# prip-lab/MSU-LatentAFIS

Measured on AMD Instinct MI355X. Metric: latent queries/sec vs 100k rolled gallery, higher is better.
Workload: dtype f32

## Files before the change

### include/afis_matcher_taps.h

```cpp
#ifndef AFIS_MATCHER_TAPS_H
#define AFIS_MATCHER_TAPS_H

#include "afis_matcher.h"

#ifdef __cplusplus
extern "C" {
#endif

int afis_debug_lut(afis_ctx* ctx, const afis_template_view* query, float* out, int32_t* n_rows);
int afis_debug_texture_rowmax(afis_ctx* ctx, const afis_template_view* query, int64_t g,
                              float* val, int32_t* arg, int32_t* n_rows);

int afis_debug_stage_list(afis_ctx* ctx, const afis_template_view* query, int64_t g, int which, int stage,
                          float* sim, int32_t* li, int32_t* ri, int32_t* n);

int afis_debug_atan2_grid(afis_ctx* ctx, int R, float* out);

int afis_debug_graph_arith(afis_ctx* ctx, unsigned long long* out8);
int afis_debug_refine_stats(afis_ctx* ctx, unsigned long long* out8, int reset);

int afis_debug_compact_stats(afis_ctx* ctx, long long* out2);

int afis_debug_rank_subjects(afis_ctx* ctx, afis_subjects* subjects, const float* scores , int n_q, int k,
                             int64_t* subject_id, float* subject_score, int64_t* best_idx);

int afis_debug_rank_hits(afis_ctx* ctx, afis_subjects* subjects, const float* scores , int n_q, float min_score, int cap,
                         int64_t* n_hits , int64_t* out_a , float* out_score , int64_t* out_b );

int afis_debug_rank_latent_hits(afis_ctx* ctx, const float* scores , int n_q, float min_score, int cap, int64_t latent_base,
                                int64_t* n_hits , int64_t* latent_idx , float* score );
int afis_debug_rank_rows(afis_ctx* ctx, afis_subset* subset, const float* scores , int n_q, int k,
                         int64_t* topk_idx , float* topk_score );
int afis_debug_transpose_stats(afis_ctx* ctx, long long* out2);
int afis_debug_expand_rows(afis_ctx* ctx, const float* cls , int n_c, int64_t m, const int32_t* row_of , const int32_t* sel ,
                           int n_q, int64_t G, float* out );

int afis_debug_phase_cycles(afis_ctx* ctx, unsigned long long* out32, int reset);

#ifdef __cplusplus
}
#endif
#endif
```

### msu-latentafis_amd/csrc/afis_device.h

```cpp
#pragma once
#include <hip/hip_runtime.h>
#include <stdint.h>

#include "score_order.h"

namespace afis {

typedef unsigned long long u64;
constexpr int kM = 16;
constexpr int kK = 256;
constexpr int kDsub = 6;
constexpr int kDes = 96;
constexpr int kTexMax = 1000;
constexpr int kTopTex = 200;
constexpr int kTopMinu = 120;
constexpr int kDistN = 50;
constexpr int kTileRows = 8;
constexpr int kTileFloats = kTileRows * kM * kK;

struct GalleryDev {
    int32_t G = 0;
    const int32_t* minu_off = nullptr;
    const short2*  minu_xy = nullptr;
    const float*   minu_ori = nullptr;
// ... 86 lines not shown
AFIS_HOST_DEVICE constexpr int rt_class_keys_per_thread(int S) { return S == 4 ? 64 : 32; }
AFIS_HOST_DEVICE inline int rt_row_stride(int S, int nR) { return S == 1 ? (((nR & 1) || nR == 128) ? nR : nR + 1) : (nR | 1); }
AFIS_HOST_DEVICE inline int rt_max_rows(int S, int nR)
{
    if (nR <= 0 || nR > rt_class_max_rolled(S)) return 0;
    int m = rt_class_keys_per_thread(S) * ((256 * S) / nR);
    const int cap = rt_class_simi_floats(S) / rt_row_stride(S, nR);
    m = m < cap ? m : cap;
    return m < rt_class_max_latent(S) ? m : rt_class_max_latent(S);
}
inline long long launch_group_latents(long long G) { if (G < 1) G = 1; const long long w = (5000000 + G / 2) / G; return w < 10 ? 10 : w > 128 ? 128 : w; }
inline void launch_group_cuts(const long long* rows_prefix, int n, int per, bool by_row_groups, int* cuts , int* n_cuts)
{
    *n_cuts = 0;
    if (n <= 0) return;
    if (per < 1) per = 1;
    if (!by_row_groups || n == 1) { for (int i = per; i < n; i += per) cuts[(*n_cuts)++] = i; cuts[(*n_cuts)++] = n; return; }
    const long long kInf = 1ll << 60, rg_rows = 768;
    long long* best = new long long[(size_t)n + 1]; int* from = new int[(size_t)n + 1]; int* cnt = new int[(size_t)n + 1];
    best[0] = 0; from[0] = 0; cnt[0] = 0;
    for (int i = 1; i <= n; ++i) {
        best[i] = kInf; from[i] = 0; cnt[i] = 0;
        for (int j = (i - per > 0 ? i - per : 0); j < i; ++j) {
            const long long c = best[j] + (rows_prefix[i] - rows_prefix[j] + rg_rows - 1) / rg_rows;
            if (c < best[i] || (c == best[i] && cnt[j] + 1 < cnt[i])) { best[i] = c; from[i] = j; cnt[i] = cnt[j] + 1; }
        }
    }
    int m = 0;
    for (int i = n; i > 0; i = from[i]) cuts[m++] = i;
    for (int a = 0, b = m - 1; a < b; ++a, --b) { const int t = cuts[a]; cuts[a] = cuts[b]; cuts[b] = t; }
    *n_cuts = m;
    delete[] best; delete[] from; delete[] cnt;
}
inline size_t minu_fb_ints(size_t n_tasks, size_t G) { return 1 + n_tasks + 8 + 3 * G; }
inline size_t minu_scratch_floats(int max_nL, int max_nR, int s3_tie_order)
{
    const size_t n = ((size_t)(max_nL > 1 ? max_nL : 1) * (size_t)(max_nR > 1 ? max_nR : 1) + 63) / 64 * 64;
    return (s3_tie_order ? 5 : 2) * n + 4096;
}
enum { kDiagFallback = 0,
       kDiagSmall = 1,
       kDiagCandsClk = 4, kDiagCandsWall = 5,
       kDiagBoundClk = 6, kDiagBoundWall = 7,
       kDiagWords = 16 };
constexpr int kTexSlabSteps = 48, kMinuSlabSteps = 32;
constexpr size_t kTexSlabWgBytes = (size_t)((kTopTex + 63) / 64) * kTexSlabSteps * 64 * 5;
constexpr size_t kMinuSlabWgBytes = (size_t)((kTopMinu + 63) / 64) * kMinuSlabSteps * 64 * 5;
inline int graph_texture_grid(long long n_tasks) { return (int)(n_tasks < 16384 ? n_tasks : 16384); }
inline int graph_minutiae_grid(long long n_tasks) { return (int)(n_tasks < 32768 ? n_tasks : 32768); }
inline size_t graph_texture_slab_bytes(long long n_tasks) { return n_tasks > 0 ? (size_t)graph_texture_grid(n_tasks) * kTexSlabWgBytes : 0; }
inline size_t graph_minutiae_slab_bytes(long long n_tasks) { return n_tasks > 0 ? (size_t)graph_minutiae_grid(n_tasks) * kMinuSlabWgBytes : 0; }
hipError_t launch_graph_texture(const QueryDev& q, const GalleryDev& g, const float* table_dist,
                                const float* rm_val, const int32_t* rm_arg, const float* rm_cv, const int32_t* rm_n, float* parts, void* slab, size_t slab_bytes, MinuCand* tap_out, int32_t* tap_n, int tap_stage, hipStream_t stream);
hipError_t launch_minu_cands(const QueryDev& q, const GalleryDev& g, float* scratch, size_t scratch_floats_per_wg, int n_wg,
                             int force_generic, MinuCand* cands, int32_t* cand_n, int32_t* fallback , int max_nL, int max_nR,
                             unsigned long long* diag , hipStream_t stream);
hipError_t launch_graph_minutiae(const QueryDev& q, const GalleryDev& g, const MinuCand* cands, const int32_t* cand_n,
                                 float* parts, short4* corr_out, int32_t* corr_n, void* slab, size_t slab_bytes, MinuCand* tap_out, int32_t* tap_n, int tap_stage, hipStream_t stream, bool join = false);
hipError_t launch_fuse(const QueryDev& q, const GalleryDev& g, const float* parts, float* scores, hipStream_t stream);

hipError_t launch_topk(const float* scores, int n_q, int G, int k, long long index_base, long long* out_idx, float* out_score, hipStream_t stream);

hipError_t launch_pq_encode(const float* des, long long n, const float* codewords, uint8_t* codes, hipStream_t stream);
hipError_t launch_fragment_tiles(const float* des, const int32_t* off, const int32_t* tile_off, int n_templates, void* frag, hipStream_t stream);
hipError_t launch_compact_ranges(const void* src, void* dst, int elem_bytes, const int32_t* old_off, const int32_t* new_off, int G, long long n_new, hipStream_t stream);
hipError_t launch_gather_ranges(const void* src, void* dst, int elem_bytes, const int32_t* src_off, const int32_t* sel, const int32_t* dst_off, int n, long long n_out, hipStream_t stream);
hipError_t launch_subset_topk_map(long long* idx, long long n_idx, const long long* map, int n_map, hipStream_t stream);
// ... 40 lines not shown
```

### msu-latentafis_amd/csrc/afis_taps.cpp

```cpp
#include "afis_ctx.h"
#include "../../include/afis_matcher_taps.h"

using namespace afis;

static int ensure_codes_cf(afis_ctx* ctx, Shard& sh, int variant)
{
    if ((variant != 6 && variant != 7) || sh.codes_cf_built) return AFIS_OK;
    const int64_t G = sh.gal.G;
    std::vector<int32_t> to((size_t)G + 1), cfb((size_t)G + 1);
    HIPCHK(ctx, hipMemcpyAsync(to.data(), sh.gal.tex_off, to.size() * 4, hipMemcpyDeviceToHost, ctx->stream));
    HIPCHK(ctx, hipStreamSynchronize(ctx->stream));
    int64_t nblk = 0;
    for (int64_t t = 0; t < G; ++t) { cfb[(size_t)t] = (int32_t)nblk; const int64_t n = to[(size_t)t + 1] - to[(size_t)t]; nblk += n > 0 ? (n + 63) / 64 + 1 : 0; }
    cfb[(size_t)G] = (int32_t)nblk;
    if (nblk > 0x7fffffff / 64) return fail(ctx, AFIS_EINVAL, "adc_variant 6 / 7: shard too large for the direct kernel's code stream; split the gallery into more shards");
    HIPCHK(ctx, upload(sh.g_tex_cf_blk, cfb, ctx->stream));
    HIPCHK(ctx, sh.g_tex_codes_cf.ensure(std::max<size_t>((size_t)nblk * 64 * 16, 16)));
    sh.gal.tex_cf_blk = sh.g_tex_cf_blk.as<int32_t>();
    sh.gal.tex_codes_cf = sh.g_tex_codes_cf.as<uint4>();
    HIPCHK(ctx, launch_codes_cf(sh.gal, sh.g_tex_codes_cf.p, ctx->stream));
    HIPCHK(ctx, hipStreamSynchronize(ctx->stream));
    sh.codes_cf_built = true;
    return AFIS_OK;
}
// ... 279 lines not shown
            HIPCHK(ctx, ctx->rm_val.ensure((size_t)d.lt_pad * 4)); HIPCHK(ctx, ctx->rm_arg.ensure((size_t)d.lt_pad * 4));
            const int av = ctx->adc_variant >= 8 ? 0 : ctx->adc_variant;
            { int rcf = ensure_codes_cf(ctx, *ctx, av); if (rcf != AFIS_OK) return rcf; }
            if (av == 6 || av == 7) { one.tex_codes_cf = ctx->gal.tex_codes_cf; one.tex_cf_blk = ctx->gal.tex_cf_blk + gidx; }
            { int rcd = direct_rowmax(ctx, d, one, av, 32, nullptr); if (rcd != AFIS_OK) return rcd; }
            HIPCHK(ctx, ctx->tex_slab.ensure(graph_texture_slab_bytes(d.nq)));
            HIPCHK(ctx, launch_graph_texture(d, one, ctx->table.as<float>(), ctx->rm_val.as<float>(), ctx->rm_arg.as<int32_t>(), nullptr, nullptr, ctx->parts.as<float>(), ctx->tex_slab.p, ctx->tex_slab.bytes,
                                             d_out.as<MinuCand>(), d_n.as<int32_t>(), stage | (ctx->s89_tie_order << 8), s));
        } else {
            slot = which - 1; cap = kTopMinu;
            const size_t per_wg = minu_scratch_floats(grp.max_nL, ctx->max_nR, ctx->s3_tie_order);
            HIPCHK(ctx, ctx->scratch.ensure(per_wg * 4 * 64));
            HIPCHK(ctx, ctx->cands.ensure(3 * (size_t)kTopMinu * sizeof(MinuCand))); HIPCHK(ctx, ctx->cand_n.ensure(12)); HIPCHK(ctx, ctx->minu_fb.ensure(minu_fb_ints(3, 1) * 4));
            HIPCHK(ctx, launch_minu_cands(d, one, ctx->scratch.as<float>(), per_wg, 64, ctx->minu_generic | (ctx->s3_tie_order << 1), ctx->cands.as<MinuCand>(), ctx->cand_n.as<int32_t>(), ctx->minu_fb.as<int32_t>(), grp.max_nL, ctx->max_nR, nullptr, s));
            HIPCHK(ctx, ctx->minu_slab.ensure(graph_minutiae_slab_bytes(3ll * d.nq)));
            HIPCHK(ctx, launch_graph_minutiae(d, one, ctx->cands.as<MinuCand>(), ctx->cand_n.as<int32_t>(), ctx->parts.as<float>(), nullptr, nullptr, ctx->minu_slab.p, ctx->minu_slab.bytes,
                                              d_out.as<MinuCand>(), d_n.as<int32_t>(), stage | (ctx->s89_tie_order << 8), s));
        }
        std::vector<MinuCand> h((size_t)3 * kTopTex); int32_t hn[3] = {-1, -1, -1};
        HIPCHK(ctx, hipMemcpyAsync(h.data(), d_out.p, h.size() * sizeof(MinuCand), hipMemcpyDeviceToHost, s));
        HIPCHK(ctx, hipMemcpyAsync(hn, d_n.p, 12, hipMemcpyDeviceToHost, s));
        HIPCHK(ctx, hipStreamSynchronize(s));
        if (ctx->res_empty[(size_t)gidx]) return AFIS_OK;
        *n = hn[slot];
        for (int t = 0; t < hn[slot]; ++t) { const MinuCand& c = h[(size_t)slot * cap + t]; sim[t] = c.sim; li[t] = c.li; ri[t] = c.ri; }
        return AFIS_OK;
    };
    rc = body();
    d_out.release(); d_n.release(); grp.release();
    return rc;
}


}
```

### msu-latentafis_amd/csrc/minu.hip

```cpp
#include "afis_device.h"
#include "stdsort_order.h"
#include <cstdlib>

namespace afis {

constexpr int kThreads = 256;
constexpr int kWaves = kThreads / 64;

#ifdef AFIS_PHASE_TIMING
__device__ u64 g_phase_cycles[32];
#define PHASE_DECL() __shared__ u64 ph_acc[32]; if (threadIdx.x < 32) ph_acc[threadIdx.x] = 0; __syncthreads()
#define PHASE_FLUSH() do { __syncthreads(); if (threadIdx.x < 32 && ph_acc[threadIdx.x]) atomicAdd(&g_phase_cycles[threadIdx.x], ph_acc[threadIdx.x]); } while (0)
#define PHASE_INIT() u64 ph_t0 = __builtin_readcyclecounter()
#define PHASE(i) do { if (threadIdx.x == 0) { const u64 ph_t1 = __builtin_readcyclecounter(); ph_acc[i] += ph_t1 - ph_t0; ph_t0 = ph_t1; } } while (0)
#else
#define PHASE_DECL() do {} while (0)
#define PHASE_FLUSH() do {} while (0)
#define PHASE_INIT() do {} while (0)
#define PHASE(i) do {} while (0)
#endif

__device__ __forceinline__ int wg_sum(int wave_total, int* s_slots , int& parity)
{
    if ((threadIdx.x & 63) == 0) s_slots[parity * kWaves + (threadIdx.x >> 6)] = wave_total;
// ... 370 lines not shown
    for (int i = tid; i < 258; i += 256) cnt[i] = 0;
    __syncthreads();
    for (int qs = tid; qs < nqs; qs += 256) { const int nL = q.lm_off[qs + 1] - q.lm_off[qs]; atomicAdd(&cnt[nL <= 0 ? 0 : min(nL, 257)], 1); }
    __syncthreads();
    if (tid == 0) { int run = 0; for (int x = 1; x <= 257; ++x) { run += cnt[x]; cnt[x] = run; } }
    __syncthreads();
    const int gi = blockIdx.x * 256 + tid;
    const bool live = gi < g.G;
    const int nR = live ? g.minu_off[gi + 1] - g.minu_off[gi] : 0;
    const int L1 = rt_max_rows(1, nR), L2 = rt_max_rows(2, nR), L4 = rt_max_rows(4, nR);
    const int c1 = live && L1 > 0 ? cnt[L1] : 0, c2 = live && L2 > 0 ? cnt[L2] : c1, c4 = live && L4 > 0 ? cnt[L4] : c2;
    const int has[3] = {c1, c2 - c1, c4 - c2};
#pragma unroll
    for (int c = 0; c < 3; ++c) {
        const u64 m = __ballot(has[c] > 0);
        if (m) {
            const int leader = __ffsll((long long)m) - 1;
            int base = 0;
            if (lane == leader) base = atomicAdd(&ctl[c], __popcll(m));
            base = __shfl(base, leader);
            if (has[c] > 0) work[(size_t)c * g.G + base + lane_prefix(m)] = gi;
        }
    }
    if (live && (nR <= 0 || cnt[0] > 0 || cnt[257] > c4)) {
        for (int qs = 0; qs < nqs; ++qs) {
            const long long task = (long long)qs * g.G + gi;
            const int nL = q.lm_off[qs + 1] - q.lm_off[qs];
            if (nR <= 0 || nL <= 0) cand_n[task] = 0;
            else if (nL > L4) { const int p = atomicAdd(&fb[0], 1); fb[1 + p] = (int32_t)task; }
        }
    }
}

template <int S, int ref_tie_order >
__global__ __launch_bounds__(256 * S, 4) void k_minu_cands_rt(QueryDev q, GalleryDev g, const float4* __restrict__ lat_frag,
                                                                const float4* __restrict__ rol_frag,
                                                                MinuCand* __restrict__ cands, int32_t* __restrict__ cand_n, int32_t* __restrict__ fb,
                                                                const int32_t* __restrict__ work ,
                                                                int32_t* __restrict__ ctl ,
                                                                unsigned long long* __restrict__ diag )
{
    typedef RtCfg<S> Cfg;
    constexpr int kT = Cfg::kT, kW = Cfg::kW, kSimi = Cfg::kSimi, kCls = S == 1 ? 0 : S == 2 ? 1 : 2;
    extern __shared__ __attribute__((aligned(16))) unsigned char rt_smem_raw[];
    RtSmem<S>& sm = *reinterpret_cast<RtSmem<S>*>(rt_smem_raw);
    PHASE_DECL();
    typedef float f32x4 __attribute__((ext_vector_type(4)));
    const int tid = threadIdx.x, lane = tid & 63;
    const int wave = __builtin_amdgcn_readfirstlane(tid >> 6);
    const int li = lane & 15, lg = lane >> 4;
    const int nqs = q.nq * 3;
    auto to_fallback = [&](long long task) { const int p = atomicAdd(&fb[0], 1); fb[1 + p] = (int32_t)task; };
    const bool sampler = diag != nullptr && blockIdx.x < 8 && wave == 0;
    unsigned long long clk0 = 0, wall0 = 0;
    if (sampler) { clk0 = __builtin_readcyclecounter(); wall0 = wall_clock64(); }
    int n_done = 0;
    const int n_work = ctl[kCls];
    const int n_split = n_work <= 0 || n_work >= 2 * (int)gridDim.x ? 1 : min(nqs, (2 * (int)gridDim.x + n_work - 1) / n_work);
    const int n_tickets = n_work * n_split;
    if (tid == 0) sm.pad_[1] = 0;
    for (;;) {
        if (tid == 0) sm.ticket = atomicAdd(&ctl[4 + kCls], 1);
        __syncthreads();
        const int wi = sm.ticket;
        __syncthreads();
        if (wi >= n_tickets) break;
        const int gi = work[(size_t)kCls * g.G + wi / n_split];
        const int tpart = wi - (wi / n_split) * n_split;
        const int qs_lo = (int)((long long)nqs * tpart / n_split), qs_hi = (int)((long long)nqs * (tpart + 1) / n_split);
        const int r0 = g.minu_off[gi], nR = g.minu_off[gi + 1] - r0;
        const int Lhi = rt_max_rows(S, nR), Llo = S == 1 ? 0 : rt_max_rows(S / 2, nR);
        const int n_jt = (nR + 15) >> 4;
        const int ld = rt_row_stride(S, nR);
        const int R = kT / nR;
        const int cr = tid / nR, cj = tid - cr * nR;
        const int n_res = min(n_jt, kW), P = kW / n_res;
        const int jt_res = wave % n_res, part = wave / n_res;
        const unsigned lane16 = (unsigned)lane * 16u;
        const char* const btiles = reinterpret_cast<const char*>(rol_frag + (size_t)g.minu_tile_off[gi] * (6 * 64));
        auto frag_at = [&](const char* base, int t, int v) -> const float4& { return *reinterpret_cast<const float4*>(base + ((unsigned)((t * 6 + v) * 1024) + lane16)); };
        float bres[24];
#pragma unroll
        for (int v = 0; v < 6; ++v) { const float4 x = frag_at(btiles, jt_res, v); bres[4 * v] = x.x; bres[4 * v + 1] = x.y; bres[4 * v + 2] = x.z; bres[4 * v + 3] = x.w; }
        auto next_in_class = [&](int from) {
            int x = from;
            for (; x < qs_hi; ++x) { const int nl = q.lm_off[x + 1] - q.lm_off[x]; if (nl > Llo && nl <= Lhi) break; }
            return x;
        };
        int pf_qs = -1, pf_n = 0;
        int qs_next = next_in_class(qs_lo);
        for (int qs = qs_next; qs < qs_hi; qs = qs_next) {
            qs_next = next_in_class(qs + 1);
            const long long task = (long long)qs * g.G + gi;
            const int l0 = q.lm_off[qs], nL = q.lm_off[qs + 1] - l0;
            const int n = nL * nR;
            if (n < kHistMinN) { if (tid == 0) to_fallback(task); continue; }
            PHASE_INIT();
            const int n_it = (nL + 15) >> 4;
            const char* const atiles = reinterpret_cast<const char*>(lat_frag + (size_t)q.lm_tile_off[qs] * (6 * 64));
            const int n_pf = pf_qs == qs ? pf_n : 0;
            const char* const a_end = reinterpret_cast<const char*>(sm.simi + kSimi);
            auto a_lds = [&](int t) { return a_end - (t + 1) * (6 * 64 * 16); };
// ... 128 lines not shown
                    for (int t = 32; t < n_rows; ++t) {
                        if (t < my_rows) {
                            const uint32_t key = approx_norm_key(sm.simi[a], sm.rowsum[i], cs);
                            const int bin = min((int)((key >> 19) & 0xfffu) - kBinBase, kSelBins - 1);
                            if (bin > 0) atomicAdd(&sm.hist[bin], 1u);
                        }
                        a += R * ld; i += R;
                    }
                }
            }
            __syncthreads();
            PHASE(29);
            if (wave == 0) {
                const uint4 h = reinterpret_cast<const uint4*>(sm.hist)[lane];
                const int s0 = (int)(h.x + h.y + h.z + h.w);
                int suf = s0;
                suf += __builtin_amdgcn_update_dpp(0, suf, 0x101, 0xf, 0xf, true);
                suf += __builtin_amdgcn_update_dpp(0, suf, 0x102, 0xf, 0xf, true);
                suf += __builtin_amdgcn_update_dpp(0, suf, 0x104, 0xf, 0xf, true);
                suf += __builtin_amdgcn_update_dpp(0, suf, 0x108, 0xf, 0xf, true);
                const int r1 = __builtin_amdgcn_readlane(suf, 16), r2 = __builtin_amdgcn_readlane(suf, 32), r3 = __builtin_amdgcn_readlane(suf, 48);
                suf += lane < 16 ? r1 + r2 + r3 : lane < 32 ? r2 + r3 : lane < 48 ? r3 : 0;
                const int a3 = suf - s0, a2 = a3 + (int)h.w, a1 = a2 + (int)h.z, a0 = a1 + (int)h.y;
                if (a3 < kTopMinu && a3 + (int)h.w >= kTopMinu) sm.thr_bin = 4 * lane + 3;
                if (a2 < kTopMinu && a2 + (int)h.z >= kTopMinu) sm.thr_bin = 4 * lane + 2;
                if (a1 < kTopMinu && a1 + (int)h.y >= kTopMinu) sm.thr_bin = 4 * lane + 1;
                if (a0 < kTopMinu && a0 + (int)h.x >= kTopMinu) sm.thr_bin = 4 * lane;
                reinterpret_cast<uint4*>(sm.hist)[lane] = make_uint4((uint32_t)a0, (uint32_t)a1, (uint32_t)a2, (uint32_t)a3);
            }
            __syncthreads();
            PHASE(30);
            const int Braw = __builtin_amdgcn_readfirstlane(sm.thr_bin);
            bool fill = false;
            if (__builtin_expect(Braw < 0 && !ref_tie_order, 0)) {
                if (tid == 0) sm.pad_[0] = 0;
                __syncthreads();
                bool tiny = false;
                {
                    const float cs2 = my_rows > 0 ? sm.colsum[cj] : 0.0f;
                    for (int t = 0; t < my_rows; ++t) {
                        const int i = cr + R * t;
                        const uint32_t key = approx_norm_key(sm.simi[i * ld + cj], sm.rowsum[i], cs2);
                        tiny |= (key & 0x7fffffffu) != 0u && (int)((key >> 19) & 0xfffu) - kBinBase <= 0;
                    }
                }
                if (tiny) sm.pad_[0] = 1;
                __syncthreads();
                fill = __builtin_amdgcn_readfirstlane(sm.pad_[0]) == 0;
            }
            if (__builtin_expect(Braw < 2 && !fill, 0)) { if (tid == 0) to_fallback(task); asm volatile("s_waitcnt vmcnt(0)" ::: "memory"); __syncthreads(); continue; }
            const int B = fill ? 0 : Braw;
            uint32_t edge = fill ? 0x80000001u + kKeySlack : 0x80000000u | ((uint32_t)(B + kBinBase) << 19);
            if (!fill) {
                const int above = (int)sm.hist[B], inbin = (int)sm.hist[B - 1] - above;
                if (__builtin_expect(above + inbin > kCandCap - 32 && B < kSelBins - 1, 0)) {
                    uint32_t* const h2 = reinterpret_cast<uint32_t*>(sm.cand);
                    if (tid < 256) h2[tid] = 0u;
                    __syncthreads();
                    const uint32_t bin_bits = edge >> 19;
                    {
                        const float cs2 = my_rows > 0 ? sm.colsum[cj] : 0.0f;
                        for (int t = 0; t < my_rows; ++t) {
                            const int i = cr + R * t;
                            const uint32_t key = approx_norm_key(sm.simi[i * ld + cj], sm.rowsum[i], cs2);
                            if ((key >> 19) == bin_bits) atomicAdd(&h2[(key >> 11) & 255u], 1u);
                        }
                    }
                    __syncthreads();
                    if (wave == 0) {
                        const int need = kTopMinu - above;
                        if (lane == 0) sm.thr_bin = 0;
                        const uint4 h = reinterpret_cast<const uint4*>(h2)[lane];
                        const int s0 = (int)(h.x + h.y + h.z + h.w);
                        int suf = s0;
                        suf += __builtin_amdgcn_update_dpp(0, suf, 0x101, 0xf, 0xf, true);
                        suf += __builtin_amdgcn_update_dpp(0, suf, 0x102, 0xf, 0xf, true);
                        suf += __builtin_amdgcn_update_dpp(0, suf, 0x104, 0xf, 0xf, true);
                        suf += __builtin_amdgcn_update_dpp(0, suf, 0x108, 0xf, 0xf, true);
                        const int r1 = __builtin_amdgcn_readlane(suf, 16), r2 = __builtin_amdgcn_readlane(suf, 32), r3 = __builtin_amdgcn_readlane(suf, 48);
                        suf += lane < 16 ? r1 + r2 + r3 : lane < 32 ? r2 + r3 : lane < 48 ? r3 : 0;
                        const int a3 = suf - s0, a2 = a3 + (int)h.w, a1 = a2 + (int)h.z, a0 = a1 + (int)h.y;
                        if (a3 < need && a3 + (int)h.w >= need) sm.thr_bin = 4 * lane + 3;
                        if (a2 < need && a2 + (int)h.z >= need) sm.thr_bin = 4 * lane + 2;
                        if (a1 < need && a1 + (int)h.y >= need) sm.thr_bin = 4 * lane + 1;
                        if (a0 < need && a0 + (int)h.x >= need) sm.thr_bin = 4 * lane;
                    }
                    __syncthreads();
                    edge |= (uint32_t)__builtin_amdgcn_readfirstlane(sm.thr_bin) << 11;
// ... 45 lines not shown
            PHASE(18);
            if (tid < n_c) {
                const u64 mine = sm.cand[tid];
                const uint32_t edge_own = 0x80000000u | ((uint32_t)(cbin + kBinBase) << 19), edge_up = edge_own + (1u << 19);
                const bool need_up = cbin + 1 < kSelBins && ke + kKeySlack >= edge_up;
                const bool need_dn = ke < edge_own + kKeySlack;
                const int lo = need_up ? (cbin + 2 < kSelBins ? (int)sm.hist[cbin + 2] & ~1 : 0) : (cbin + 1 < kSelBins ? (int)sm.hist[cbin + 1] & ~1 : 0);
                const int hi = cbin <= B ? n_c : need_dn ? (cbin - 1 > B ? (int)sm.hist[cbin - 1] : n_c) : (int)sm.hist[cbin];
                int r = lo;
                const ulonglong2* c2 = reinterpret_cast<const ulonglong2*>(sm.cand);
                for (int k = lo; k < hi; k += 8) {
                    const ulonglong2 k0 = c2[(k >> 1)], k1 = c2[(k >> 1) + 1], k2 = c2[(k >> 1) + 2], k3 = c2[(k >> 1) + 3];
                    r += (int)(k0.x > mine) + (int)(k0.y > mine) + (int)(k1.x > mine) + (int)(k1.y > mine) + (int)(k2.x > mine) + (int)(k2.y > mine) + (int)(k3.x > mine) + (int)(k3.y > mine);
                }
                if (r < kTopMinu) {
                    MinuCand cd; cd.sim = sm.simi[ci * ld + cj2]; cd.li = (short)ci; cd.ri = (short)cj2;
                    cands[(size_t)task * kTopMinu + r] = cd;
                }
                if (ref_tie_order && r <= kTopMinu) sm.cand_e[r] = ke;
            }
            if (fill && wave == 0) {
                int rank = n_c;
                for (int e0 = 0; e0 < n && rank < kTopMinu; e0 += 64) {
                    const int e = e0 + lane;
                    const int i = e / nR, j = e - i * nR;
                    const bool z = e < n && sm.simi[i * ld + j] == 0.0f;
                    const u64 zm = __ballot(z);
                    const int r = rank + lane_prefix(zm);
                    if (z && r < kTopMinu) { MinuCand cd; cd.sim = 0.0f; cd.li = (short)i; cd.ri = (short)j; cands[(size_t)task * kTopMinu + r] = cd; }
                    rank += (int)__popcll(zm);
                }
            }
            if (tid == 0) cand_n[task] = kTopMinu;
            ++n_done;
            __syncthreads();
            if (ref_tie_order) {
                if (tid + 1 < min(n_c, kTopMinu + 1) && sm.cand_e[tid] == sm.cand_e[tid + 1]) sm.pad_[1] = 1;
                __syncthreads();
                if (tid == 0 && sm.pad_[1] != 0) { sm.pad_[1] = 0; to_fallback(task); }
            }
            PHASE(20);
        }
    }
    if (diag != nullptr && tid == 0) {
        if (n_done) atomicAdd(&diag[kDiagSmall + kCls], (unsigned long long)n_done);
        if (sampler) { atomicAdd(&diag[kDiagCandsClk], (unsigned long long)__builtin_readcyclecounter() - clk0); atomicAdd(&diag[kDiagCandsWall], (unsigned long long)wall_clock64() - wall0); }
    }
    PHASE_FLUSH();
}

template <int S, int REF>
static hipError_t launch_rt_class_t(const QueryDev& q, const GalleryDev& g, MinuCand* cands, int32_t* cand_n, int32_t* fallback, int32_t* work, int32_t* ctl, unsigned long long* diag, hipStream_t stream)
{
    hipError_t e = hipFuncSetAttribute(reinterpret_cast<const void*>(k_minu_cands_rt<S, REF>), hipFuncAttributeMaxDynamicSharedMemorySize, (int)sizeof(RtSmem<S>));
    if (e != hipSuccess) return e;
    const int per_cu = 4 / S;
#ifndef AFIS_RT_GRID_CAP
#define AFIS_RT_GRID_CAP 0
#endif
    const int full = (AFIS_RT_GRID_CAP > 0 && S == 1) ? AFIS_RT_GRID_CAP : 256 * per_cu;
    const int grid = g.G < full ? g.G : full;
    hipLaunchKernelGGL((k_minu_cands_rt<S, REF>), dim3(grid), dim3(256 * S), sizeof(RtSmem<S>), stream, q, g, q.lm_frag, g.minu_frag, cands, cand_n, fallback, work, ctl, diag);
    return hipGetLastError();
}
template <int S>
static hipError_t launch_rt_class(const QueryDev& q, const GalleryDev& g, MinuCand* cands, int32_t* cand_n, int32_t* fallback, int32_t* work, int32_t* ctl, unsigned long long* diag, int ref_tie_order, hipStream_t stream)
{
    return ref_tie_order ? launch_rt_class_t<S, 1>(q, g, cands, cand_n, fallback, work, ctl, diag, stream) : launch_rt_class_t<S, 0>(q, g, cands, cand_n, fallback, work, ctl, diag, stream);
}

hipError_t launch_minu_cands(const QueryDev& q, const GalleryDev& g, float* scratch, size_t scratch_floats_per_wg, int n_wg,
                             int force_generic, MinuCand* cands, int32_t* cand_n, int32_t* fallback, int max_nL, int max_nR, unsigned long long* diag, hipStream_t stream)
{
    const long long n_tasks = (long long)q.nq * 3 * g.G;
    if (n_tasks <= 0) return hipSuccess;
    if (n_tasks > 0x7ffffff0LL) return hipErrorInvalidValue;
    hipError_t e;
    const int ref_tie_order = (force_generic >> 1) & 1;
    force_generic &= 1;
    if (!force_generic) {
        int32_t* ctl = fallback + 1 + n_tasks;
        int32_t* work = ctl + 8;
        e = hipMemsetAsync(fallback, 0, sizeof(int32_t), stream);
        if (e != hipSuccess) return e;
        e = hipMemsetAsync(ctl, 0, 8 * sizeof(int32_t), stream);
        if (e != hipSuccess) return e;
        hipLaunchKernelGGL(k_minu_classify, dim3((g.G + 255) / 256), dim3(256), 0, stream, q, g, work, ctl, cand_n, fallback);
        e = hipGetLastError();
        if (e != hipSuccess) return e;
        e = launch_rt_class<1>(q, g, cands, cand_n, fallback, work, ctl, diag, ref_tie_order, stream);
        if (e != hipSuccess) return e;
        const int mr = max_nR < 256 ? (max_nR > 0 ? max_nR : 1) : 256;
        if (max_nL > rt_class_max_latent(1) || max_nR > rt_class_max_rolled(1)) {
            e = launch_rt_class<2>(q, g, cands, cand_n, fallback, work, ctl, diag, ref_tie_order, stream);
            if (e != hipSuccess) return e;
            if (max_nR > rt_class_max_rolled(2) || max_nL > rt_max_rows(2, mr)) {
                e = launch_rt_class<4>(q, g, cands, cand_n, fallback, work, ctl, diag, ref_tie_order, stream);
                if (e != hipSuccess) return e;
            }
        }
    }
    e = hipFuncSetAttribute(reinterpret_cast<const void*>(k_minu_cands), hipFuncAttributeMaxDynamicSharedMemorySize, (int)sizeof(MinuSmem));
    if (e != hipSuccess) return e;
    const int grid = (int)(n_tasks < n_wg ? n_tasks : n_wg);
    const size_t smem = ref_tie_order ? sizeof(MinuSmem) : offsetof(MinuSmem, order);
    hipLaunchKernelGGL(k_minu_cands, dim3(grid), dim3(kThreads), smem, stream, q, g, scratch, scratch_floats_per_wg, cands, cand_n,
                       force_generic ? (const int32_t*)nullptr : fallback, diag, ref_tie_order);
    return hipGetLastError();
}

__global__ __launch_bounds__(256) void k_fuse(QueryDev q, GalleryDev g, const float* __restrict__ parts, float* __restrict__ scores)
{
    const long long idx = (long long)blockIdx.x * 256 + threadIdx.x;
    const long long n = (long long)q.nq * g.G;
    if (idx >= n) return;
    const int qi = (int)(idx / g.G), gi = (int)(idx - (long long)qi * g.G);
    if (q.status[qi] != 0 || g.empty[gi]) { scores[idx] = -1.0f; return; }
    const float* p = parts + (size_t)idx * 4;
    const int slot = q.tex_slot[qi];
    const float tex = p[3];
    const float a0 = slot == 0 ? tex : p[0];
    const float a1 = slot == 1 ? tex : p[1];
    const float a2 = slot == 2 ? tex : p[2];
    const float a28 = slot == 28 ? tex : 0.0f;
    float f = a0 + a1;
    f = f + a2;
    scores[idx] = (float)((double)f + (double)a28 * 0.3);
}

constexpr int kTopkThreads = 1024;
__global__ __launch_bounds__(kTopkThreads) void k_topk(const float* __restrict__ scores, int G, int k, long long index_base,
                                                      long long* __restrict__ out_idx, float* __restrict__ out_score)
{
// ... 62 lines not shown
```

### msu-latentafis_amd/host/matcher.py

```python
from __future__ import annotations

import ctypes as C
import glob
import os
from typing import List, Optional, Sequence, Tuple

import numpy as np

from .templates import Codebook, FPTemplate, read_latent, read_rolled

_HERE = os.path.dirname(os.path.abspath(__file__))
LIB_PATH = os.path.join(os.path.dirname(_HERE), "csrc", "libafis_hip.so")
TEST_LIB_PATH = os.path.join(os.path.dirname(_HERE), "csrc", "libafis_hip_test.so")


class AfisError(RuntimeError):
    pass


CASE_SUM, CASE_MAX = 0, 1


class MinutiaeView(C.Structure):
    _fields_ = [("n", C.c_int32), ("x", C.POINTER(C.c_int16)), ("y", C.POINTER(C.c_int16)), ("ori", C.POINTER(C.c_float)),
                ("des_len", C.c_int32), ("des", C.POINTER(C.c_float))]


class TextureView(C.Structure):
    _fields_ = [("n", C.c_int32), ("x", C.POINTER(C.c_int16)), ("y", C.POINTER(C.c_int16)), ("ori", C.POINTER(C.c_float)),
                ("des_len", C.c_int32), ("des", C.POINTER(C.c_float)), ("codes", C.POINTER(C.c_uint8))]


class TemplateView(C.Structure):
    _fields_ = [("n_minu", C.c_int32), ("minu", C.POINTER(MinutiaeView)), ("n_tex", C.c_int32), ("tex", C.POINTER(TextureView))]


class Timing(C.Structure):
    _fields_ = [("lut_ms", C.c_float), ("adc_ms", C.c_float), ("tex_tail_ms", C.c_float), ("minu_ms", C.c_float), ("fuse_ms", C.c_float), ("topk_ms", C.c_float),
                ("total_ms", C.c_float), ("adc_launches", C.c_int32), ("adc_lookups", C.c_int64), ("pairs", C.c_int64), ("adc_bound_ms", C.c_float), ("adc_refine_ms", C.c_float),
                ("cands_ms", C.c_float), ("minu_graph_ms", C.c_float), ("launch_groups", C.c_int32), ("overlapped_groups", C.c_int32),
                ("minu_tasks", C.c_int64), ("minu_fallback_tasks", C.c_int64), ("minu_tasks_small", C.c_int64), ("minu_tasks_medium", C.c_int64), ("minu_tasks_large", C.c_int64),
                ("bound_clock_ghz", C.c_float), ("cands_clock_ghz", C.c_float)]


EXPORTS = ["afis_create", "afis_create_from_codebook", "afis_device_info", "afis_destroy", "afis_last_error", "afis_gallery_add", "afis_gallery_add_dat", "afis_gallery_add_dat_batch", "afis_gallery_reserve",
           "afis_gallery_add_packed", "afis_gallery_commit", "afis_gallery_size", "afis_gallery_reopen", "afis_gallery_remove", "afis_gallery_export", "afis_gallery_save", "afis_gallery_load",
           "afis_gallery_file_info", "afis_gallery_file_names", "afis_rank_list", "afis_search", "afis_search_dat", "afis_queries_upload",
           "afis_subset_create", "afis_subset_free", "afis_search_subset", "afis_search_subset_resident",
           "afis_subjects_create", "afis_subjects_free", "afis_rank_subjects", "afis_rank_hits", "afis_rank_subject_hits", "afis_queries_upload_reserved", "afis_rank_latent_hits",
           "afis_rank_case_hits", "afis_rank_case_subject_hits",
           "afis_labels_create", "afis_labels_free", "afis_rank_hits_filtered", "afis_rank_subject_hits_filtered",
           "afis_rank_case_hits_filtered", "afis_rank_case_subject_hits_filtered", "afis_rank_latent_hits_filtered", "afis_search_eligible",
           "afis_rank_positions", "afis_rank_subject_positions", "afis_count_before",
           "afis_search_resident", "afis_queries_free", "afis_correspondences", "afis_match_all_templates", "afis_pq_encode", "afis_encode_rolled_dat", "afis_get_timing", "afis_get_timing2", "afis_set_option", "afis_get_option"]
TAP_EXPORTS = ["afis_debug_lut", "afis_debug_texture_rowmax", "afis_debug_stage_list", "afis_debug_phase_cycles", "afis_debug_atan2_grid", "afis_debug_graph_arith", "afis_debug_refine_stats", "afis_debug_compact_stats", "afis_debug_rank_subjects", "afis_debug_rank_hits", "afis_debug_rank_latent_hits",
               "afis_debug_transpose_stats", "afis_debug_rank_rows", "afis_debug_expand_rows"]


def load_library(path: str = LIB_PATH) -> C.CDLL:
    if not os.path.exists(path):
        raise AfisError(f"{path} not found: build it with `make -C msu-latentafis_amd/csrc` (hipcc, gfx950). There is no CPU fallback.")
    lib = C.CDLL(path)
    vp, i32p, i64p, fp = C.c_void_p, C.POINTER(C.c_int32), C.POINTER(C.c_int64), C.POINTER(C.c_float)
    lib.afis_create.argtypes = [C.POINTER(vp), fp, C.c_int, C.c_int, C.c_int, C.c_int]
    lib.afis_create_from_codebook.argtypes = [C.POINTER(vp), C.c_char_p, C.c_size_t, C.c_int]
    lib.afis_destroy.argtypes = [vp]; lib.afis_destroy.restype = None
    lib.afis_last_error.argtypes = [vp]; lib.afis_last_error.restype = C.c_char_p
    lib.afis_rank_list.argtypes = [C.POINTER(C.c_float), C.c_int64, C.c_int, C.c_int, C.POINTER(C.c_int64), C.POINTER(C.c_float)]
    lib.afis_gallery_add.argtypes = [vp, C.POINTER(TemplateView), C.c_int]
    lib.afis_gallery_add_dat.argtypes = [vp, C.c_char_p, C.c_size_t, i32p]
    lib.afis_gallery_reserve.argtypes = [vp, C.c_int64]
    if hasattr(lib, "afis_gallery_add_dat_batch"):
        lib.afis_gallery_add_dat_batch.argtypes = [vp, C.POINTER(C.c_char_p), C.POINTER(C.c_size_t), C.c_int64, i32p]
    lib.afis_gallery_add_packed.argtypes = [vp, C.c_int64, i64p, C.POINTER(C.c_int16), C.POINTER(C.c_int16), fp, fp,
                                            i64p, C.POINTER(C.c_int16), C.POINTER(C.c_int16), fp, C.POINTER(C.c_uint8)]
    lib.afis_gallery_commit.argtypes = [vp, C.c_int64]
    lib.afis_gallery_save.argtypes = [vp, C.c_char_p, C.POINTER(C.c_char_p)]
    lib.afis_gallery_load.argtypes = [vp, C.c_char_p, C.c_int64, C.c_int64]
    lib.afis_gallery_file_info.argtypes = [C.c_char_p, i64p, i64p, i64p, i32p]
    lib.afis_gallery_file_names.argtypes = [C.c_char_p, C.c_int64, C.c_int64, C.c_char_p, C.c_size_t, C.POINTER(C.c_size_t)]
    lib.afis_gallery_size.argtypes = [vp]; lib.afis_gallery_size.restype = C.c_int64
    if hasattr(lib, "afis_gallery_reopen"):
        lib.afis_gallery_reopen.argtypes = [vp]
        lib.afis_gallery_remove.argtypes = [vp, i64p, C.c_int64]
        lib.afis_gallery_export.argtypes = [vp, C.c_char_p, C.POINTER(C.c_char_p)]
    lib.afis_search.argtypes = [vp, C.POINTER(TemplateView), C.c_int, fp, fp, i32p, C.c_int, i64p, fp]
    lib.afis_search_dat.argtypes = [vp, C.POINTER(C.c_char_p), C.POINTER(C.c_size_t), C.c_int, fp, fp, i32p, C.c_int, i64p, fp]
    lib.afis_queries_upload.argtypes = [vp, C.POINTER(TemplateView), C.c_int, C.POINTER(vp)]
    lib.afis_search_resident.argtypes = [vp, vp, fp, fp, i32p, C.c_int, i64p, fp]
# ... 21 lines not shown
        lib.afis_labels_free.argtypes = [vp, vp]; lib.afis_labels_free.restype = None
        lib.afis_rank_hits_filtered.argtypes = [vp, vp, u64p, i64p, i64p, C.c_int, C.c_float, C.c_int, i64p, i64p, fp]
        lib.afis_rank_subject_hits_filtered.argtypes = [vp, vp, vp, u64p, i64p, i64p, C.c_int, C.c_float, C.c_int, i64p, i64p, fp, i64p]
    if hasattr(lib, "afis_rank_case_hits_filtered"):
        lib.afis_rank_case_hits_filtered.argtypes = [vp, vp, u64p, i64p, i64p, i64p, C.c_int, C.c_int, C.c_int64, C.c_float, C.c_int, i64p, i64p, i64p, fp]
        lib.afis_rank_case_subject_hits_filtered.argtypes = [vp, vp, vp, u64p, i64p, i64p, i64p, C.c_int, C.c_int, C.c_int64, C.c_float, C.c_int, i64p, i64p, i64p, fp]
        lib.afis_rank_latent_hits_filtered.argtypes = [vp, vp, u64p, i64p, i64p, C.c_int64, C.c_float, C.c_int, C.c_int64, i64p, i64p, fp]
    if hasattr(lib, "afis_search_eligible"):
        lib.afis_search_eligible.argtypes = [vp, vp, C.POINTER(C.c_uint64), C.POINTER(TemplateView), C.c_int, fp, i32p]
    if hasattr(lib, "afis_rank_positions"):
        u64p = C.POINTER(C.c_uint64)
        lib.afis_rank_positions.argtypes = [vp, vp, u64p, i64p, i64p, C.c_int, C.c_int64, i32p, i64p, i32p, i64p, fp]
        lib.afis_rank_subject_positions.argtypes = [vp, vp, vp, u64p, i64p, i64p, C.c_int, C.c_int64, i32p, i64p, i32p, i64p, fp, i64p]
        lib.afis_count_before.argtypes = [vp, vp, u64p, i64p, i64p, C.c_int, C.c_int64, i32p, fp, i64p, i64p]
    lib.afis_correspondences.argtypes = [vp, vp, i64p, C.c_int, i32p, C.POINTER(C.c_int16)]
    lib.afis_queries_free.argtypes = [vp, vp]; lib.afis_queries_free.restype = None
    lib.afis_match_all_templates.argtypes = [vp, vp, fp, i32p, i32p]
    lib.afis_pq_encode.argtypes = [vp, fp, C.c_int64, C.POINTER(C.c_uint8)]
    lib.afis_encode_rolled_dat.argtypes = [vp, C.c_char_p, C.c_size_t, C.c_void_p, C.c_size_t, C.POINTER(C.c_size_t), i32p]
    lib.afis_get_timing.argtypes = [vp, C.POINTER(Timing)]
    if hasattr(lib, "afis_get_timing2"):
        lib.afis_get_timing2.argtypes = [vp, C.POINTER(Timing), C.c_size_t]
    lib.afis_set_option.argtypes = [vp, C.c_char_p, C.c_int64]
    if hasattr(lib, "afis_device_info"):
        lib.afis_device_info.argtypes = [C.c_int, C.c_char_p, C.c_size_t, C.c_char_p, C.c_size_t, C.c_char_p, C.c_size_t, i32p]
    if hasattr(lib, "afis_get_option"):
        lib.afis_get_option.argtypes = [vp, C.c_char_p, i64p]
    if hasattr(lib, "afis_debug_stage_list"):
        lib.afis_debug_stage_list.argtypes = [vp, vp, C.c_int64, C.c_int, C.c_int, fp, i32p, i32p, i32p]
        lib.afis_debug_lut.argtypes = [vp, C.POINTER(TemplateView), fp, i32p]
        lib.afis_debug_texture_rowmax.argtypes = [vp, C.POINTER(TemplateView), C.c_int64, fp, i32p, i32p]
        lib.afis_debug_phase_cycles.argtypes = [vp, C.POINTER(C.c_uint64), C.c_int]
        lib.afis_debug_atan2_grid.argtypes = [vp, C.c_int, fp]
    if hasattr(lib, "afis_debug_graph_arith"):
        lib.afis_debug_graph_arith.argtypes = [vp, C.POINTER(C.c_ulonglong)]
    if hasattr(lib, "afis_debug_compact_stats"):
        lib.afis_debug_compact_stats.argtypes = [vp, C.POINTER(C.c_longlong)]
    if hasattr(lib, "afis_debug_refine_stats"):
        lib.afis_debug_refine_stats.argtypes = [vp, C.POINTER(C.c_ulonglong), C.c_int]
    if hasattr(lib, "afis_debug_rank_subjects"):
        lib.afis_debug_rank_subjects.argtypes = [vp, vp, fp, C.c_int, C.c_int, i64p, fp, i64p]
    if hasattr(lib, "afis_debug_rank_hits"):
        lib.afis_debug_rank_hits.argtypes = [vp, vp, fp, C.c_int, C.c_float, C.c_int, i64p, i64p, fp, i64p]
    if hasattr(lib, "afis_debug_rank_latent_hits"):
        lib.afis_debug_rank_latent_hits.argtypes = [vp, fp, C.c_int, C.c_float, C.c_int, C.c_int64, i64p, i64p, fp]
        lib.afis_debug_transpose_stats.argtypes = [vp, C.POINTER(C.c_longlong)]
    if hasattr(lib, "afis_debug_rank_rows"):
        lib.afis_debug_rank_rows.argtypes = [vp, vp, fp, C.c_int, C.c_int, i64p, fp]
    if hasattr(lib, "afis_debug_expand_rows"):
        lib.afis_debug_expand_rows.argtypes = [vp, fp, C.c_int, C.c_int64, i32p, i32p, C.c_int, C.c_int64, fp]
    return lib


def _ptr(a: np.ndarray, t):
    return a.ctypes.data_as(C.POINTER(t))


class _Views:

    def __init__(self, templates: Sequence[FPTemplate]):
        self.keep = []
        self.arr = (TemplateView * max(1, len(templates)))()
        for i, t in enumerate(templates):
            mv = (MinutiaeView * max(1, len(t.minu)))()
            for j, m in enumerate(t.minu):
                x = np.ascontiguousarray(m.x, np.int16); y = np.ascontiguousarray(m.y, np.int16)
# ... 492 lines not shown

    def phase_cycles(self, reset: bool = True):
        out = (C.c_uint64 * 32)()
        self._chk(self._tap("afis_debug_phase_cycles")(self.ctx, out, 1 if reset else 0))
        return list(out)

    def debug_atan2_grid(self, R: int) -> np.ndarray:
        out = np.empty((2 * R + 1, 2 * R + 1), np.float32)
        self._chk(self._tap("afis_debug_atan2_grid")(self.ctx, R, _ptr(out, C.c_float)))
        return out

    def debug_graph_arith(self) -> list:
        out = (C.c_ulonglong * 8)()
        self._chk(self._tap("afis_debug_graph_arith")(self.ctx, out))
        return list(out)

    def refine_stats(self, reset: bool = True) -> dict:
        out = (C.c_ulonglong * 8)()
        self._chk(self._tap("afis_debug_refine_stats")(self.ctx, out, 1 if reset else 0))
        return dict(zip(("pairs", "rows", "rows_evaluated", "cells_evaluated", "rows_evaluated_in_full", "bound_violations"), list(out)[:6]))

    def compact_stats(self):
        out = (C.c_longlong * 2)()
        self._chk(self._tap("afis_debug_compact_stats")(self.ctx, out))
        return int(out[0]), int(out[1])

    def debug_stage_list(self, latent: FPTemplate, g: int, which: int, stage: int):
        v = _Views([latent])
        sim = np.zeros(200, np.float32); li = np.zeros(200, np.int32); ri = np.zeros(200, np.int32); n = C.c_int32(0)
        self._chk(self._tap("afis_debug_stage_list")(self.ctx, v.arr, g, which, stage, _ptr(sim, C.c_float), _ptr(li, C.c_int32), _ptr(ri, C.c_int32), C.byref(n)))
        if n.value < 0:
            return None
        return sim[:n.value], li[:n.value], ri[:n.value]

    def debug_lut(self, latent: FPTemplate) -> np.ndarray:
        v = _Views([latent])
        n = latent.tex[0].n if latent.tex else 0
        out = np.empty((max(n, 1), 16, 256), np.float32); nr = C.c_int32(0)
        self._chk(self._tap("afis_debug_lut")(self.ctx, v.arr, _ptr(out, C.c_float), C.byref(nr)))
        return out[:nr.value]

    def debug_texture_rowmax(self, latent: FPTemplate, g: int):
        v = _Views([latent])
        val = np.zeros(1000, np.float32); arg = np.zeros(1000, np.int32); nr = C.c_int32(0)
        self._chk(self._tap("afis_debug_texture_rowmax")(self.ctx, v.arr, g, _ptr(val, C.c_float), _ptr(arg, C.c_int32), C.byref(nr)))
        return val[:nr.value], arg[:nr.value]

    def load_gallery_dir(self, rolled_path: str) -> List[str]:
        if os.path.isfile(rolled_path):
            self.gallery_load(rolled_path)
            self.gallery_files = self.gallery_file_names(rolled_path)
            self.gallery_commit(0)
            return self.gallery_files
        files = [os.path.join(rolled_path, f) for f in os.listdir(rolled_path) if os.path.splitext(f)[1] == ".dat"]
        for f in files:
            with open(f, "rb") as fh:
                self.gallery_add_dat(fh.read())
        self.gallery_files = files
        self.gallery_commit(0)
        return files

    def One2List_matching(self, latent_template_file: str, score_path: str, top: int = 24) -> int:
        with open(latent_template_file, "rb") as f:
            buf = f.read()
        stem = os.path.splitext(os.path.basename(latent_template_file))[0]
        _, parsed = read_latent(buf)
# ... 50 lines not shown
```

Before: 52.06.

## Defer rare slow-path minutiae tasks to separate RARE kernel passes

The main rt candidate kernel no longer handles the rare slow paths (no positive threshold bin, crowded bin) inline. It pushes those tasks to a rare list, and follow-up launches of a RARE template variant process them one per block with a static stride. This is meant to remove divergent, long-running slow-path work from the common fast kernel and improve load balance, at the cost of extra kernel launches and a larger work buffer. A debug tap for reading candidate lists is also added.

```diff
diff --git a/include/afis_matcher_taps.h b/include/afis_matcher_taps.h
--- a/include/afis_matcher_taps.h
+++ b/include/afis_matcher_taps.h
@@ -13,6 +13,8 @@
 
 int afis_debug_stage_list(afis_ctx* ctx, const afis_template_view* query, int64_t g, int which, int stage,
                           float* sim, int32_t* li, int32_t* ri, int32_t* n);
+
+int afis_debug_search_cands(afis_ctx* ctx, int64_t task0, int64_t n_tasks, float* sim, int32_t* li, int32_t* ri, int32_t* n);
 
 int afis_debug_atan2_grid(afis_ctx* ctx, int R, float* out);
 
diff --git a/msu-latentafis_amd/csrc/afis_device.h b/msu-latentafis_amd/csrc/afis_device.h
--- a/msu-latentafis_amd/csrc/afis_device.h
+++ b/msu-latentafis_amd/csrc/afis_device.h
@@ -142,7 +142,7 @@
     *n_cuts = m;
     delete[] best; delete[] from; delete[] cnt;
 }
-inline size_t minu_fb_ints(size_t n_tasks, size_t G) { return 1 + n_tasks + 8 + 3 * G; }
+inline size_t minu_fb_ints(size_t n_tasks, size_t G) { return 1 + n_tasks + 8 + 3 * G + n_tasks; }
 inline size_t minu_scratch_floats(int max_nL, int max_nR, int s3_tie_order)
 {
     const size_t n = ((size_t)(max_nL > 1 ? max_nL : 1) * (size_t)(max_nR > 1 ? max_nR : 1) + 63) / 64 * 64;
diff --git a/msu-latentafis_amd/csrc/afis_taps.cpp b/msu-latentafis_amd/csrc/afis_taps.cpp
--- a/msu-latentafis_amd/csrc/afis_taps.cpp
+++ b/msu-latentafis_amd/csrc/afis_taps.cpp
@@ -335,4 +335,19 @@
 }
 
 
-}
+int afis_debug_search_cands(afis_ctx* ctx, int64_t task0, int64_t n_tasks, float* sim, int32_t* li, int32_t* ri, int32_t* n)
+{
+    if (!ctx || !sim || !li || !ri || !n || task0 < 0 || n_tasks <= 0) return fail(ctx, AFIS_EINVAL, "afis_debug_search_cands: bad argument");
+    const size_t end = (size_t)task0 + (size_t)n_tasks;
+    if (end * kTopMinu * sizeof(MinuCand) > ctx->cands.bytes || end * 4 > ctx->cand_n.bytes) return fail(ctx, AFIS_EINVAL, "afis_debug_search_cands: tasks beyond the last search's lists");
+    HIPCHK(ctx, hipSetDevice(ctx->device));
+    std::vector<MinuCand> h((size_t)n_tasks * kTopMinu);
+    HIPCHK(ctx, hipStreamSynchronize(ctx->stream));
+    HIPCHK(ctx, hipMemcpy(h.data(), ctx->cands.as<MinuCand>() + (size_t)task0 * kTopMinu, h.size() * sizeof(MinuCand), hipMemcpyDeviceToHost));
+    HIPCHK(ctx, hipMemcpy(n, ctx->cand_n.as<int32_t>() + task0, (size_t)n_tasks * 4, hipMemcpyDeviceToHost));
+    for (size_t t = 0; t < h.size(); ++t) { sim[t] = h[t].sim; li[t] = h[t].li; ri[t] = h[t].ri; }
+    return AFIS_OK;
+}
+
+
+}
diff --git a/msu-latentafis_amd/csrc/minu.hip b/msu-latentafis_amd/csrc/minu.hip
--- a/msu-latentafis_amd/csrc/minu.hip
+++ b/msu-latentafis_amd/csrc/minu.hip
@@ -426,12 +426,14 @@
     }
 }
 
-template <int S, int ref_tie_order >
+template <int S, int ref_tie_order ,
+          int RARE >
 __global__ __launch_bounds__(256 * S, 4) void k_minu_cands_rt(QueryDev q, GalleryDev g, const float4* __restrict__ lat_frag,
                                                                 const float4* __restrict__ rol_frag,
                                                                 MinuCand* __restrict__ cands, int32_t* __restrict__ cand_n, int32_t* __restrict__ fb,
                                                                 const int32_t* __restrict__ work ,
                                                                 int32_t* __restrict__ ctl ,
+                                                                int32_t* __restrict__ rare ,
                                                                 unsigned long long* __restrict__ diag )
 {
     typedef RtCfg<S> Cfg;
@@ -445,23 +447,33 @@
     const int li = lane & 15, lg = lane >> 4;
     const int nqs = q.nq * 3;
     auto to_fallback = [&](long long task) { const int p = atomicAdd(&fb[0], 1); fb[1 + p] = (int32_t)task; };
-    const bool sampler = diag != nullptr && blockIdx.x < 8 && wave == 0;
+    auto to_rare = [&](long long task) { const int p = atomicAdd(&ctl[3], 1); rare[p] = (int32_t)task; };
+    const bool sampler = !RARE && diag != nullptr && blockIdx.x < 8 && wave == 0;
     unsigned long long clk0 = 0, wall0 = 0;
     if (sampler) { clk0 = __builtin_readcyclecounter(); wall0 = wall_clock64(); }
     int n_done = 0;
-    const int n_work = ctl[kCls];
-    const int n_split = n_work <= 0 || n_work >= 2 * (int)gridDim.x ? 1 : min(nqs, (2 * (int)gridDim.x + n_work - 1) / n_work);
+    const int n_work = RARE ? ctl[3] : ctl[kCls];
+    const int n_split = RARE || n_work <= 0 || n_work >= 2 * (int)gridDim.x ? 1 : min(nqs, (2 * (int)gridDim.x + n_work - 1) / n_work);
     const int n_tickets = n_work * n_split;
     if (tid == 0) sm.pad_[1] = 0;
+    int rare_i = blockIdx.x;
     for (;;) {
-        if (tid == 0) sm.ticket = atomicAdd(&ctl[4 + kCls], 1);
-        __syncthreads();
-        const int wi = sm.ticket;
-        __syncthreads();
-        if (wi >= n_tickets) break;
-        const int gi = work[(size_t)kCls * g.G + wi / n_split];
-        const int tpart = wi - (wi / n_split) * n_split;
-        const int qs_lo = (int)((long long)nqs * tpart / n_split), qs_hi = (int)((long long)nqs * (tpart + 1) / n_split);
+        int wi, gi, qs_lo, qs_hi;
+        if (RARE) {
+            wi = rare_i; rare_i += (int)gridDim.x;
+            if (wi >= n_tickets) break;
+            const int t = rare[wi];
+            qs_lo = t / g.G; gi = t - qs_lo * g.G; qs_hi = qs_lo + 1;
+        } else {
+            if (tid == 0) sm.ticket = atomicAdd(&ctl[4 + kCls], 1);
+            __syncthreads();
+            wi = sm.ticket;
+            __syncthreads();
+            if (wi >= n_tickets) break;
+            gi = work[(size_t)kCls * g.G + wi / n_split];
+            const int tpart = wi - (wi / n_split) * n_split;
+            qs_lo = (int)((long long)nqs * tpart / n_split); qs_hi = (int)((long long)nqs * (tpart + 1) / n_split);
+        }
         const int r0 = g.minu_off[gi], nR = g.minu_off[gi + 1] - r0;
         const int Lhi = rt_max_rows(S, nR), Llo = S == 1 ? 0 : rt_max_rows(S / 2, nR);
         const int n_jt = (nR + 15) >> 4;
@@ -656,7 +668,8 @@
             PHASE(30);
             const int Braw = __builtin_amdgcn_readfirstlane(sm.thr_bin);
             bool fill = false;
-            if (__builtin_expect(Braw < 0 && !ref_tie_order, 0)) {
+            if (!RARE && Braw < 0 && !ref_tie_order) { if (tid == 0) to_rare(task); asm volatile("s_waitcnt vmcnt(0)" ::: "memory"); __syncthreads(); continue; }
+            if (RARE && Braw < 0 && !ref_tie_order) {
                 if (tid == 0) sm.pad_[0] = 0;
                 __syncthreads();
                 bool tiny = false;
@@ -677,7 +690,9 @@
             uint32_t edge = fill ? 0x80000001u + kKeySlack : 0x80000000u | ((uint32_t)(B + kBinBase) << 19);
             if (!fill) {
                 const int above = (int)sm.hist[B], inbin = (int)sm.hist[B - 1] - above;
-                if (__builtin_expect(above + inbin > kCandCap - 32 && B < kSelBins - 1, 0)) {
+                const bool crowded = above + inbin > kCandCap - 32 && B < kSelBins - 1;
+                if (!RARE && __builtin_expect(crowded, 0)) { if (tid == 0) to_rare(task); asm volatile("s_waitcnt vmcnt(0)" ::: "memory"); __syncthreads(); continue; }
+                if (RARE && crowded) {
                     uint32_t* const h2 = reinterpret_cast<uint32_t*>(sm.cand);
                     if (tid < 256) h2[tid] = 0u;
                     __syncthreads();
@@ -789,13 +804,14 @@
                 }
             }
             if (tid == 0) cand_n[task] = kTopMinu;
-            ++n_done;
-            __syncthreads();
+            __syncthreads();
+            bool redo = false;
             if (ref_tie_order) {
                 if (tid + 1 < min(n_c, kTopMinu + 1) && sm.cand_e[tid] == sm.cand_e[tid + 1]) sm.pad_[1] = 1;
                 __syncthreads();
-                if (tid == 0 && sm.pad_[1] != 0) { sm.pad_[1] = 0; to_fallback(task); }
-            }
+                if (tid == 0 && sm.pad_[1] != 0) { sm.pad_[1] = 0; to_fallback(task); redo = true; }
+            }
+            if (!redo) ++n_done;
             PHASE(20);
         }
     }
@@ -806,10 +822,10 @@
     PHASE_FLUSH();
 }
 
-template <int S, int REF>
+template <int S, int REF, int RARE>
 static hipError_t launch_rt_class_t(const QueryDev& q, const GalleryDev& g, MinuCand* cands, int32_t* cand_n, int32_t* fallback, int32_t* work, int32_t* ctl, unsigned long long* diag, hipStream_t stream)
 {
-    hipError_t e = hipFuncSetAttribute(reinterpret_cast<const void*>(k_minu_cands_rt<S, REF>), hipFuncAttributeMaxDynamicSharedMemorySize, (int)sizeof(RtSmem<S>));
+    hipError_t e = hipFuncSetAttribute(reinterpret_cast<const void*>(k_minu_cands_rt<S, REF, RARE>), hipFuncAttributeMaxDynamicSharedMemorySize, (int)sizeof(RtSmem<S>));
     if (e != hipSuccess) return e;
     const int per_cu = 4 / S;
 #ifndef AFIS_RT_GRID_CAP
@@ -817,13 +833,13 @@
 #endif
     const int full = (AFIS_RT_GRID_CAP > 0 && S == 1) ? AFIS_RT_GRID_CAP : 256 * per_cu;
     const int grid = g.G < full ? g.G : full;
-    hipLaunchKernelGGL((k_minu_cands_rt<S, REF>), dim3(grid), dim3(256 * S), sizeof(RtSmem<S>), stream, q, g, q.lm_frag, g.minu_frag, cands, cand_n, fallback, work, ctl, diag);
+    hipLaunchKernelGGL((k_minu_cands_rt<S, REF, RARE>), dim3(grid), dim3(256 * S), sizeof(RtSmem<S>), stream, q, g, q.lm_frag, g.minu_frag, cands, cand_n, fallback, work, ctl, work + 3 * (size_t)g.G, diag);
     return hipGetLastError();
 }
-template <int S>
+template <int S, int RARE>
 static hipError_t launch_rt_class(const QueryDev& q, const GalleryDev& g, MinuCand* cands, int32_t* cand_n, int32_t* fallback, int32_t* work, int32_t* ctl, unsigned long long* diag, int ref_tie_order, hipStream_t stream)
 {
-    return ref_tie_order ? launch_rt_class_t<S, 1>(q, g, cands, cand_n, fallback, work, ctl, diag, stream) : launch_rt_class_t<S, 0>(q, g, cands, cand_n, fallback, work, ctl, diag, stream);
+    return ref_tie_order ? launch_rt_class_t<S, 1, RARE>(q, g, cands, cand_n, fallback, work, ctl, diag, stream) : launch_rt_class_t<S, 0, RARE>(q, g, cands, cand_n, fallback, work, ctl, diag, stream);
 }
 
 hipError_t launch_minu_cands(const QueryDev& q, const GalleryDev& g, float* scratch, size_t scratch_floats_per_wg, int n_wg,
@@ -845,17 +861,17 @@
         hipLaunchKernelGGL(k_minu_classify, dim3((g.G + 255) / 256), dim3(256), 0, stream, q, g, work, ctl, cand_n, fallback);
         e = hipGetLastError();
         if (e != hipSuccess) return e;
-        e = launch_rt_class<1>(q, g, cands, cand_n, fallback, work, ctl, diag, ref_tie_order, stream);
+        e = launch_rt_class<1, 0>(q, g, cands, cand_n, fallback, work, ctl, diag, ref_tie_order, stream);
         if (e != hipSuccess) return e;
         const int mr = max_nR < 256 ? (max_nR > 0 ? max_nR : 1) : 256;
-        if (max_nL > rt_class_max_latent(1) || max_nR > rt_class_max_rolled(1)) {
-            e = launch_rt_class<2>(q, g, cands, cand_n, fallback, work, ctl, diag, ref_tie_order, stream);
-            if (e != hipSuccess) return e;
-            if (max_nR > rt_class_max_rolled(2) || max_nL > rt_max_rows(2, mr)) {
-                e = launch_rt_class<4>(q, g, cands, cand_n, fallback, work, ctl, diag, ref_tie_order, stream);
-                if (e != hipSuccess) return e;
-            }
-        }
+        const bool medium = max_nL > rt_class_max_latent(1) || max_nR > rt_class_max_rolled(1);
+        const bool large = medium && (max_nR > rt_class_max_rolled(2) || max_nL > rt_max_rows(2, mr));
+        if (medium) { e = launch_rt_class<2, 0>(q, g, cands, cand_n, fallback, work, ctl, diag, ref_tie_order, stream); if (e != hipSuccess) return e; }
+        if (large) { e = launch_rt_class<4, 0>(q, g, cands, cand_n, fallback, work, ctl, diag, ref_tie_order, stream); if (e != hipSuccess) return e; }
+        e = launch_rt_class<1, 1>(q, g, cands, cand_n, fallback, work, ctl, diag, ref_tie_order, stream);
+        if (e != hipSuccess) return e;
+        if (medium) { e = launch_rt_class<2, 1>(q, g, cands, cand_n, fallback, work, ctl, diag, ref_tie_order, stream); if (e != hipSuccess) return e; }
+        if (large) { e = launch_rt_class<4, 1>(q, g, cands, cand_n, fallback, work, ctl, diag, ref_tie_order, stream); if (e != hipSuccess) return e; }
     }
     e = hipFuncSetAttribute(reinterpret_cast<const void*>(k_minu_cands), hipFuncAttributeMaxDynamicSharedMemorySize, (int)sizeof(MinuSmem));
     if (e != hipSuccess) return e;
diff --git a/msu-latentafis_amd/host/matcher.py b/msu-latentafis_amd/host/matcher.py
--- a/msu-latentafis_amd/host/matcher.py
+++ b/msu-latentafis_amd/host/matcher.py
@@ -54,7 +54,7 @@
            "afis_rank_positions", "afis_rank_subject_positions", "afis_count_before",
            "afis_search_resident", "afis_queries_free", "afis_correspondences", "afis_match_all_templates", "afis_pq_encode", "afis_encode_rolled_dat", "afis_get_timing", "afis_get_timing2", "afis_set_option", "afis_get_option"]
 TAP_EXPORTS = ["afis_debug_lut", "afis_debug_texture_rowmax", "afis_debug_stage_list", "afis_debug_phase_cycles", "afis_debug_atan2_grid", "afis_debug_graph_arith", "afis_debug_refine_stats", "afis_debug_compact_stats", "afis_debug_rank_subjects", "afis_debug_rank_hits", "afis_debug_rank_latent_hits",
-               "afis_debug_transpose_stats", "afis_debug_rank_rows", "afis_debug_expand_rows"]
+               "afis_debug_transpose_stats", "afis_debug_rank_rows", "afis_debug_expand_rows", "afis_debug_search_cands"]
 
 
 def load_library(path: str = LIB_PATH) -> C.CDLL:
@@ -142,6 +142,8 @@
         lib.afis_debug_texture_rowmax.argtypes = [vp, C.POINTER(TemplateView), C.c_int64, fp, i32p, i32p]
         lib.afis_debug_phase_cycles.argtypes = [vp, C.POINTER(C.c_uint64), C.c_int]
         lib.afis_debug_atan2_grid.argtypes = [vp, C.c_int, fp]
+    if hasattr(lib, "afis_debug_search_cands"):
+        lib.afis_debug_search_cands.argtypes = [vp, C.c_int64, C.c_int64, fp, i32p, i32p, i32p]
     if hasattr(lib, "afis_debug_graph_arith"):
         lib.afis_debug_graph_arith.argtypes = [vp, C.POINTER(C.c_ulonglong)]
     if hasattr(lib, "afis_debug_compact_stats"):
@@ -700,6 +702,11 @@
         if n.value < 0:
             return None
         return sim[:n.value], li[:n.value], ri[:n.value]
+
+    def debug_search_cands(self, task0: int, n_tasks: int):
+        sim = np.zeros((n_tasks, 120), np.float32); li = np.zeros((n_tasks, 120), np.int32); ri = np.zeros((n_tasks, 120), np.int32); n = np.zeros(n_tasks, np.int32)
+        self._chk(self._tap("afis_debug_search_cands")(self.ctx, C.c_int64(task0), C.c_int64(n_tasks), _ptr(sim, C.c_float), _ptr(li, C.c_int32), _ptr(ri, C.c_int32), _ptr(n, C.c_int32)))
+        return n, sim, li, ri
 
     def debug_lut(self, latent: FPTemplate) -> np.ndarray:
         v = _Views([latent])
```

Result: no change. 52.08 (median of 2 runs) (+0.0%).
